# VITA-Group/FasterSeg

Measured on NVIDIA H100. Metric: fasterseg_student_fps_1024x2048, higher is better.
Workload: dtype fp16

## Files before the change

fasterseg_b200/_lib.py:

```python
import ctypes as C
import os

_HERE = os.path.dirname(os.path.abspath(__file__))
LIB_PATH = os.path.join(_HERE, "libfsb200.so")

FSB_CONV_RELU = 1
FSB_CONV_AFFINE = 2
FSB_CONV_FORCE_DIRECT = 4
FSB_CONV_STATS = 8
FSB_CONV_OUT_F32 = 16
FSB_ACT_IN_F32 = 32
FSB_CONV_X_DOWN2 = 64
FSB_CONV_Y_UP2 = 128
ABI_VERSION = 2


class FsbError(RuntimeError):
    pass


class ConvDesc(C.Structure):
    _fields_ = [(n, C.c_int32) for n in ("N", "H", "W", "Cin", "Cout", "ksize", "stride", "pad", "dil", "off_h", "off_w",
                                         "Ho", "Wo", "x_cstride", "y_cstride")] + [("flags", C.c_uint32), ("stats_C", C.c_int32),
                                                                                    ("stats_off", C.c_int32)]


class BnSel(C.Structure):
    _fields_ = [("gamma", C.c_void_p), ("beta", C.c_void_p), ("running_mean", C.c_void_p), ("running_var", C.c_void_p),
                ("num_batches_tracked", C.c_void_p), ("dgamma", C.c_void_p), ("dbeta", C.c_void_p), ("C", C.c_int32),
                ("reserved", C.c_int32)]


_P = C.c_void_p
_SIGS = {
    "fsb_abi_version": (C.c_int, []),
    "fsb_last_error_string": (C.c_char_p, []),
    "fsb_device_info": (C.c_int, [C.POINTER(C.c_int)] * 3),
    "fsb_set_pdl": (C.c_int, [C.c_int]),
    "fsb_set_option": (C.c_int, [C.c_char_p, C.c_int]),
    "fsb_get_option": (C.c_int, [C.c_char_p]),
    "fsb_conv_kernel_id": (C.c_int, [C.POINTER(ConvDesc), _P, C.c_int]),
    "fsb_conv_stats_rows": (C.c_int, [C.POINTER(ConvDesc)]),
    "fsb_stat_rows": (C.c_int, [C.c_int64]),
    "fsb_wsum_rows": (C.c_int, [C.c_int64, C.c_int]),
    "fsb_rowsum": (C.c_int, [C.c_int, _P, C.c_int, C.c_int, _P, _P]),
    "fsb_debug_set_buffer": (C.c_int, [_P]),
    "fsb_conv_packed_bytes": (C.c_size_t, [C.POINTER(ConvDesc)]),
    "fsb_pack_conv_weight": (C.c_int, [C.POINTER(ConvDesc), _P, C.c_int64, C.c_int64, _P, _P]),
    "fsb_bn_fold": (C.c_int, [C.c_int, _P, _P, _P, _P, C.c_float, _P, _P, _P, _P]),
    "fsb_conv_fwd": (C.c_int, [C.POINTER(ConvDesc), _P, _P, _P, _P, _P, _P, _P]),
    "fsb_stem_conv_nchw": (C.c_int, [C.c_int] * 4 + [_P, C.c_int, _P, _P, _P, _P, C.c_int, C.c_uint32, _P]),
    "fsb_stem_conv_u8hwc": (C.c_int, [C.c_int] * 4 + [_P, _P, _P, _P, _P, _P, C.c_int, C.c_uint32, _P]),
    "fsb_confusion_matrix": (C.c_int, [C.c_int64, _P, _P, C.c_int, C.c_int, _P, _P]),
    "fsb_bilinear_fwd": (C.c_int, [C.c_int] * 6 + [_P, C.c_int, _P, C.c_int, C.c_uint32, _P]),
    "fsb_upsample_logits_nchw": (C.c_int, [C.c_int] * 6 + [_P, C.c_int, _P, C.c_int, _P]),
    "fsb_upsample_argmax": (C.c_int, [C.c_int] * 6 + [_P, C.c_int, _P, _P]),
    "fsb_nearest_fwd": (C.c_int, [C.c_int] * 6 + [_P, C.c_int, _P, C.c_int, _P]),
    "fsb_upsample_logits_nearest_nchw": (C.c_int, [C.c_int] * 6 + [_P, C.c_int, _P, C.c_int, _P]),
    "fsb_upsample_argmax_nearest": (C.c_int, [C.c_int] * 6 + [_P, C.c_int, _P, _P]),
    "fsb_nchw_to_nhwc_f16": (C.c_int, [C.c_int] * 4 + [_P, C.c_int, _P, C.c_int, _P]),
    "fsb_nhwc_f16_to_nchw": (C.c_int, [C.c_int] * 4 + [_P, C.c_int, _P, C.c_int, _P]),
    "fsb_copy_channels": (C.c_int, [C.c_int64, C.c_int, _P, C.c_int, _P, C.c_int, _P]),
    "fsb_bn_stats": (C.c_int, [C.c_int64, C.c_int, _P, C.c_int, _P, _P]),
    "fsb_bn_finalize": (C.c_int, [C.c_int, _P, C.c_int, C.c_int, C.c_double, _P, _P, C.c_float, C.c_float, _P, _P, _P, _P, _P, _P, _P]),
    "fsb_affine_act": (C.c_int, [C.c_int64, C.c_int, _P, C.c_int, _P, _P, _P, C.c_int, C.c_uint32, _P]),
    "fsb_bn_bwd_reduce": (C.c_int, [C.c_int64, C.c_int, _P, C.c_int, _P, C.c_int, _P, C.c_int, C.c_int, _P, _P, C.c_int, _P, _P]),
    "fsb_bn_bwd_apply": (C.c_int, [C.c_int64, C.c_int, _P, C.c_int, _P, C.c_int, _P, C.c_int, C.c_int, _P, _P, _P, _P, C.c_double,
                                   C.c_int, _P, C.c_int, _P, _P, C.c_float, C.c_int, _P]),
    "fsb_bn_finalize_sel": (C.c_int, [C.c_int, _P, C.c_int, C.c_int, C.c_double, C.c_float, C.c_float, _P, _P, _P, _P, _P, _P, C.c_int, _P]),
    "fsb_affine_act_sel": (C.c_int, [C.c_int64, C.c_int, _P, C.c_int, _P, _P, _P, C.c_int, C.c_uint32, _P, _P, C.c_int, _P]),
    "fsb_bn_bwd_reduce_sel": (C.c_int, [C.c_int64, C.c_int, _P, C.c_int, _P, C.c_int, _P, C.c_int, C.c_int, _P, _P, C.c_int, _P,
                                        _P, _P, C.c_int, _P]),
    "fsb_bn_bwd_apply_sel": (C.c_int, [C.c_int64, C.c_int, _P, C.c_int, _P, C.c_int, _P, C.c_int, C.c_int, _P, _P, _P, _P, C.c_double,
                                       C.c_int, _P, C.c_int, C.c_float, _P, _P, C.c_int, _P]),
    "fsb_relu_bwd": (C.c_int, [C.c_int64, C.c_int, _P, C.c_int, _P, C.c_int, _P, C.c_int, _P]),
# ... 78 lines not shown
```

fasterseg_b200/csrc/api.cu:

```cuda
#include <stdlib.h>
#include <string.h>

#include <mutex>

#include "fsb_internal.h"

namespace fsb {

static thread_local char g_err[512] = "";
thread_local cudaError_t g_launch_err = cudaSuccess;

int set_error(int code, const char* msg) {
  snprintf(g_err, sizeof(g_err), "%s", msg);
  return code;
}
int set_cuda_error(cudaError_t e, const char* where) {
  snprintf(g_err, sizeof(g_err), "%s: %s (%s)", where, cudaGetErrorString(e), cudaGetErrorName(e));
  return FSB_ERR_CUDA;
}

static int g_pdl = -1;
bool pdl_enabled() {
  if (g_pdl < 0) {
    const char* e = getenv("FSB_PDL");
// ... 154 lines not shown
  return FSB_OK;
}

static int find_opt(const char* name) {
  if (!name) return -1;
  for (int i = 0; i < OPT_COUNT; ++i)
    if (strcmp(name, kOptNames[i]) == 0) return i;
  return -1;
}
int fsb_set_option(const char* name, int value) {
  const int i = find_opt(name);
  if (i < 0) return set_error(FSB_ERR_INVALID, "fsb_set_option: unknown option");
  opt(static_cast<Opt>(i));
  g_opts[i] = value;
  return FSB_OK;
}
int fsb_get_option(const char* name) {
  const int i = find_opt(name);
  return i < 0 ? -1 : opt(static_cast<Opt>(i));
}

int fsb_conv_stats_rows(const fsb_conv_desc* d) {
  if (check_desc(d)) return 0;
  if ((d->flags & FSB_CONV_FORCE_DIRECT) || !conv_tc_supported(d)) return stat_rows(static_cast<int64_t>(d->N) * d->Ho * d->Wo);
  return conv_tc_m_tiles(d);
}
int fsb_conv_kernel_id(const fsb_conv_desc* d, const void* y, int with_stats) {
  if (check_desc(d)) return -1;
  if ((d->flags & FSB_CONV_FORCE_DIRECT) || !conv_tc_supported(d)) return 0;
  (void)y;
  (void)with_stats;
  return conv_tc_strip(d) ? 2 : 1;
}
int fsb_stat_rows(int64_t pixels) { return stat_rows(pixels); }
int fsb_wsum_rows(int64_t pixels, int C) { return wsum_rows(pixels, C); }
int fsb_rowsum(int L, const float* src, int rows, int stride, float* out, void* stream) {
  if (L <= 0 || rows <= 0 || !src || !out || stride < L) return set_error(FSB_ERR_INVALID, "rowsum: bad argument");
  return rowsum_launch(L, src, rows, stride, out, static_cast<cudaStream_t>(stream));
}

int fsb_debug_set_buffer(void* dev_u64x128) {
  g_dbg_buffer = static_cast<unsigned long long*>(dev_u64x128);
  return FSB_OK;
}

int fsb_loss_logp_fwd(int N, int C, int Hi, int Wi, int Ho, int Wo, const void* logits, int cstride, const int64_t* target,
                      int ignore_label, float* logp_t, float* lse, void* stream) {
  return loss_logp_fwd_launch(N, C, Hi, Wi, Ho, Wo, logits, cstride, reinterpret_cast<const long long*>(target), ignore_label, logp_t, lse,
                              static_cast<cudaStream_t>(stream));
}
size_t fsb_kth_workspace_bytes(void) { return kth_workspace_bytes(); }
int fsb_kth_smallest_f32(const float* x, int64_t n, int64_t k, float* out, void* workspace, void* stream) {
  return kth_smallest_launch(x, n, k, out, workspace, static_cast<cudaStream_t>(stream));
}
int fsb_loss_rows(void) { return loss_rows(); }
int fsb_ohem_reduce(const float* logp_t, const int64_t* target, int64_t n, int ignore_label, int C, const float* thr, float* partial,
                    float* out2, void* stream) {
  return ohem_reduce_launch(logp_t, reinterpret_cast<const long long*>(target), n, ignore_label, C, thr, partial, out2,
                            static_cast<cudaStream_t>(stream));
}
int fsb_loss_ce_bwd(int N, int C, int Hi, int Wi, int Ho, int Wo, const void* logits, int cstride, const int64_t* target,
                    int ignore_label, const float* lse, const float* logp_t, const float* thr, const float* coef, void* dlogits,
                    int dcs, float gscale, int accumulate, void* stream) {
  return loss_ce_bwd_launch(N, C, Hi, Wi, Ho, Wo, logits, cstride, reinterpret_cast<const long long*>(target), ignore_label, lse, logp_t, thr,
                            coef, dlogits, dcs, gscale, accumulate, static_cast<cudaStream_t>(stream));
}
// ... 245 lines not shown
```

fasterseg_b200/csrc/conv_tc.cu:

```cuda
#include "fsb_common.cuh"
#include "fsb_internal.h"

namespace fsb {

constexpr int kTileM = 128;
constexpr int kMaxStages = 8;
constexpr int kThreads = 256;
constexpr int kAccLd = kTileM + 4;

struct ConvTcParams {
  CUtensorMap tmap_a[4];
  CUtensorMap tmap_b;
  CUtensorMap tmap_y[2];
  int tma_store;
  int tail_w;
  int taps;
  int tap_map[9];
  int tap_dh[9];
  int tap_dw[9];
  int tap_widx[9];
  int k_chunks;
  int Ho, Wo;
  int tiles_w, tiles_h;
  int tw, th;
  int win_pitch, win_rows;
  int win_sbo;
  int win_half;
  int win_stride;
  int m_half, m_grp;
  int Cout;
  int stages;
  int y_cstride;
  uint32_t flags;
  const float* scale;
  const float* shift;
  __half* y;
  float* stats;
  int stats_C;
  int stats_off;
};
// ... 8 lines not shown
__host__ __device__ constexpr uint32_t conv_tc_out_bytes() { return static_cast<uint32_t>((NT + 63) / 64) * kTileM * 128; }
template <int NT>
__host__ __device__ constexpr uint32_t conv_tc_epilogue_bytes() { return conv_tc_out_bytes<NT>() + static_cast<uint32_t>(NT) * kAccLd * 4; }


template <int BK, int NT, bool WIN, bool UP2>
__device__ __forceinline__ void conv_tc_body(const ConvTcParams& p, const CUtensorMap* tmap_up, int y_reps) {
  extern __shared__ uint8_t smem_raw[];
  __shared__ __align__(8) uint64_t full_bar[kMaxStages];
  __shared__ __align__(8) uint64_t empty_bar[kMaxStages];
  __shared__ __align__(8) uint64_t win_full[2];
  __shared__ __align__(8) uint64_t win_empty[2];
  __shared__ float s_scale[NT];
  __shared__ float s_shift[NT];

  pdl_launch_dependents();
  const int warp = threadIdx.x >> 5;
  const int lane = threadIdx.x & 31;
  constexpr uint32_t kABytes = kTileM * BK * 2;
  constexpr uint32_t kStageBytes = WIN ? NT * BK * 2 : kABytes + NT * BK * 2;
  static_assert(!WIN || BK == 64, "windows are 128B-swizzled 64-channel rows");
  uint8_t* smem = reinterpret_cast<uint8_t*>((reinterpret_cast<uintptr_t>(smem_raw) + 1023) & ~uintptr_t(1023));

  int t = blockIdx.x;
  const int tile_w = t % p.tiles_w;
  t /= p.tiles_w;
  const int tile_h = t % p.tiles_h;
  const int img = t / p.tiles_h;
  const int w0 = tile_w * p.tw;
  const int h0 = tile_h * p.th;
  const int n0 = blockIdx.y * NT;
  const int k_iters = p.taps * p.k_chunks;

  if (warp == 0 && lane == 0) {
    tma_prefetch_desc(&p.tmap_a[0]);
    tma_prefetch_desc(&p.tmap_b);
    for (int s = 0; s < p.stages; ++s) {
      mbar_init(&full_bar[s], 1);
      mbar_init(&empty_bar[s], 4);
    }
    for (int w = 0; w < 2; ++w) {
      mbar_init(&win_full[w], 1);
      mbar_init(&win_empty[w], 4);
    }
    mbar_fence_init();
  }
  pdl_wait();
  for (int c = threadIdx.x; c < NT; c += kThreads) {
    const int ch = n0 + c;
    const bool ok = ch < p.Cout;
    s_scale[c] = (ok && (p.flags & FSB_CONV_AFFINE) && p.scale) ? p.scale[ch] : 1.0f;
    s_shift[c] = (ok && (p.flags & FSB_CONV_AFFINE) && p.shift) ? p.shift[ch] : 0.0f;
  }
  __syncthreads();

  if (WIN && warp == 0) {
    uint8_t* bring = smem + 2 * p.win_stride;
    const uint32_t win_bytes = static_cast<uint32_t>(p.win_rows * p.win_pitch) * 128u;
    RingPos rp, rw;
    for (int kc = 0; kc < p.k_chunks; ++kc) {
      mbar_wait_inline(&win_empty[rw.s], rw.phase ^ 1u);
      if (elect_one()) {
        mbar_arrive_expect_tx(&win_full[rw.s], win_bytes);
        tma_load_4d(smem + rw.s * p.win_stride, &p.tmap_a[0], &win_full[rw.s], kc * BK, w0 + p.tap_dw[0], h0 + p.tap_dh[0], img);
      }
      __syncwarp();
      rw.advance(2);
      for (int tap = 0; tap < 9; ++tap) {
        mbar_wait_inline(&empty_bar[rp.s], rp.phase ^ 1u);
        if (elect_one()) {
          mbar_arrive_expect_tx(&full_bar[rp.s], kStageBytes);
          tma_load_3d(bring + rp.s * kStageBytes, &p.tmap_b, &full_bar[rp.s], kc * BK, n0, tap);
        }
        __syncwarp();
        rp.advance(p.stages);
      }
    }
  } else if (warp == 0) {
    RingPos rp;
    uint8_t* sa = smem;
    for (int tap = 0; tap < p.taps; ++tap) {
      const CUtensorMap* ma = &p.tmap_a[p.tap_map[tap]];
      const int cw = w0 + p.tap_dw[tap];
      const int chh = h0 + p.tap_dh[tap];
      const int wi = p.tap_widx[tap];
      for (int kc = 0; kc < p.k_chunks; ++kc) {
        mbar_wait_inline(&empty_bar[rp.s], rp.phase ^ 1u);
        if (elect_one()) {
          mbar_arrive_expect_tx(&full_bar[rp.s], kStageBytes);
          tma_load_4d(sa, ma, &full_bar[rp.s], kc * BK, cw, chh, img);
          tma_load_3d(sa + kABytes, &p.tmap_b, &full_bar[rp.s], kc * BK, n0, wi);
        }
        __syncwarp();
        sa += kStageBytes;
        rp.advance(p.stages);
        if (rp.s == 0) sa = smem;
      }
    }
  } else if (warp >= 4) {
    const int tw = threadIdx.x - 128;
    float acc[2][NT / 2];
#pragma unroll
    for (int h = 0; h < 2; ++h)
#pragma unroll
      for (int i = 0; i < NT / 2; ++i) acc[h][i] = 0.f;
    const uint32_t sa0 = smem_u32(smem);
    const uint64_t da0 = wgmma_desc_kmajor(sa0, BK * 2);
    const uint64_t db0 = wgmma_desc_kmajor(sa0 + kABytes, BK * 2);
    constexpr uint32_t kHalf = (64 * BK * 2) >> 4;
    if constexpr (WIN) {
      const uint64_t dw0 = wgmma_desc(sa0, 16, p.win_sbo, 128);
      const uint64_t dbr = wgmma_desc_kmajor(sa0 + 2 * p.win_stride, 128);
      const uint64_t whalf = static_cast<uint64_t>(p.win_half * 8);
      RingPos rp, rw;
      int prev = -1, prev_w = -1;
      for (int kc = 0; kc < p.k_chunks; ++kc) {
        mbar_wait_inline(&win_full[rw.s], rw.phase);
        const uint64_t dwin = dw0 + static_cast<uint64_t>(rw.s * (p.win_stride >> 4));
        for (int tap = 0; tap < 9; ++tap) {
          const int r = tap / 3, sx = tap - 3 * r;
          mbar_wait_inline(&full_bar[rp.s], rp.phase);
          wgmma_fence();
          const uint64_t da = dwin + static_cast<uint64_t>((r * p.win_pitch + sx) * 8);
          const uint64_t db = dbr + static_cast<uint64_t>(rp.s * (kStageBytes >> 4));
#pragma unroll
          for (int k = 0; k < BK / 16; ++k) {
            wgmma_f16<NT, 0>(acc[0], da + static_cast<uint64_t>(2 * k), db + static_cast<uint64_t>(2 * k));
            wgmma_f16<NT, 0>(acc[1], da + whalf + static_cast<uint64_t>(2 * k), db + static_cast<uint64_t>(2 * k));
          }
          wgmma_commit();
          wgmma_wait<1>();
          if (prev >= 0 && lane == 0) mbar_arrive(&empty_bar[prev]);
          if (tap == 0 && prev_w >= 0 && lane == 0) mbar_arrive(&win_empty[prev_w]);
// ... 15 lines not shown
        const uint64_t da = da0 + doff + static_cast<uint64_t>(2 * k), db = db0 + doff + static_cast<uint64_t>(2 * k);
        wgmma_f16<NT, 0>(acc[0], da, db);
        wgmma_f16<NT, 0>(acc[1], da + kHalf, db);
      }
      wgmma_commit();
      wgmma_wait<1>();
      if (prev >= 0 && lane == 0) mbar_arrive(&empty_bar[prev]);
      prev = rp.s;
      doff += kStageBytes >> 4;
      rp.advance(p.stages);
      if (rp.s == 0) doff = 0;
    }
    }
    wgmma_wait<0>();
    float* s_acc = reinterpret_cast<float*>(smem + conv_tc_out_bytes<NT>());
    named_bar_sync(1, 128);
    if constexpr (WIN) {
      const int row0 = wgmma_row(tw, 0);
      const int m0 = (row0 >> 3) * p.m_grp + (row0 & 7);
#pragma unroll
      for (int h = 0; h < 2; ++h) {
        float* s_h = s_acc + h * p.m_half + m0;
#pragma unroll
        for (int i = 0; i < NT / 2; ++i) s_h[wgmma_col(tw, i) * kAccLd + ((i >> 1) & 1) * p.m_grp] = acc[h][i];
      }
    } else {
#pragma unroll
      for (int h = 0; h < 2; ++h)
#pragma unroll
        for (int i = 0; i < NT / 2; ++i) s_acc[wgmma_col(tw, i) * kAccLd + 64 * h + wgmma_row(tw, i)] = acc[h][i];
    }
    named_bar_sync(1, 128);

    const int q = warp & 3;
    const int m = q * 32 + lane;
    const int oh = h0 + m / p.tw;
    const int ow = w0 + m % p.tw;
    const bool pix_ok = (oh < p.Ho) && (ow < p.Wo);
    __half* yrow = p.y + (static_cast<size_t>(img) * p.Ho * p.Wo + static_cast<size_t>(oh) * p.Wo + ow) * p.y_cstride + n0;
    const bool out_f32 = (p.flags & FSB_CONV_OUT_F32) != 0;
    float* yrow32 = reinterpret_cast<float*>(p.y) +
                    (static_cast<size_t>(img) * p.Ho * p.Wo + static_cast<size_t>(oh) * p.Wo + ow) * p.y_cstride + n0;
    const bool vec_ok = out_f32 ? ((reinterpret_cast<uintptr_t>(yrow32) & 15) == 0) : ((reinterpret_cast<uintptr_t>(yrow) & 15) == 0);
    const bool relu = (p.flags & FSB_CONV_RELU) != 0;
    const bool do_stats = (p.flags & FSB_CONV_STATS) != 0 && p.stats != nullptr;
    float* s_stat = reinterpret_cast<float*>(smem);
    for (int c0 = 0; c0 < NT; c0 += 64) {
      const int nb = min(4, (NT - c0) >> 4);
#pragma unroll
      for (int b = 0; b < 4; ++b) {
      if (b >= nb) break;
      const int c = c0 + 16 * b;
      float f[16];
#pragma unroll
      for (int j = 0; j < 16; ++j) f[j] = s_acc[(c + j) * kAccLd + m];
      if (do_stats) {
#pragma unroll
        for (int j = 0; j < 16; ++j) {
          float a = pix_ok ? f[j] : 0.f;
          float b = a * a;
#pragma unroll
          for (int o = 16; o > 0; o >>= 1) {
            a += __shfl_xor_sync(0xffffffffu, a, o);
            b += __shfl_xor_sync(0xffffffffu, b, o);
          }
          if (lane == 0) {
            s_stat[(q * 2 + 0) * NT + c + j] = a;
// ... 34 lines not shown
        if (NT - c0 >= 64) {
          *reinterpret_cast<uint4*>(slab + m * 128 + ((ch16 ^ (m & 7)) << 4)) = o0;
          *reinterpret_cast<uint4*>(slab + m * 128 + (((ch16 + 1) ^ (m & 7)) << 4)) = o1;
        } else {
          uint8_t* row = slab + m * (p.tail_w * 2) + (ch16 << 4);
          *reinterpret_cast<uint4*>(row) = o0;
          *reinterpret_cast<uint4*>(row + 16) = o1;
        }
      } else if (pix_ok) {
        const int remaining = p.Cout - (n0 + c);
        if (remaining >= 16 && vec_ok) {
          uint4 o0, o1;
          o0.x = pack_half2(f[0], f[1]);
          o0.y = pack_half2(f[2], f[3]);
          o0.z = pack_half2(f[4], f[5]);
          o0.w = pack_half2(f[6], f[7]);
          o1.x = pack_half2(f[8], f[9]);
          o1.y = pack_half2(f[10], f[11]);
          o1.z = pack_half2(f[12], f[13]);
          o1.w = pack_half2(f[14], f[15]);
          uint4* dst = reinterpret_cast<uint4*>(yrow + c);
          dst[0] = o0;
          dst[1] = o1;
        } else {
#pragma unroll
          for (int j = 0; j < 16; ++j)
            if (j < remaining) yrow[c + j] = __float2half_rn(f[j]);
        }
      }
      }
      if (p.tma_store) {
        fence_proxy_async_smem();
        named_bar_sync(1, 128);
        if (warp == 4 && lane == 0) {
          const bool full = (NT - c0) >= 64;
          tma_store_4d(&p.tmap_y[full ? 0 : 1], smem + static_cast<size_t>(c0 >> 6) * (kTileM * 128), n0 + c0, w0, h0, img);
          if constexpr (UP2)
            for (int l = 1; l < y_reps; ++l)
              tma_store_4d(&tmap_up[2 * l - 2 + (full ? 0 : 1)], smem + static_cast<size_t>(c0 >> 6) * (kTileM * 128), n0 + c0, w0,
                           h0, img);
          tma_store_commit();
        }
      }
    }
    if (p.tma_store && warp == 4 && lane == 0) tma_store_wait_read();
    if (do_stats) {
      named_bar_sync(2, 128);
      float* row = p.stats + static_cast<size_t>(blockIdx.x) * 2 * p.stats_C + p.stats_off;
      for (int ch = static_cast<int>(threadIdx.x) - 128; ch < NT; ch += 128) {
        if (n0 + ch >= p.Cout) continue;
        float a = s_stat[0 * NT + ch], b = s_stat[1 * NT + ch];
#pragma unroll
        for (int w = 1; w < 4; ++w) {
          a += s_stat[(w * 2 + 0) * NT + ch];
          b += s_stat[(w * 2 + 1) * NT + ch];
        }
        row[n0 + ch] = a;
        row[p.stats_C + n0 + ch] = b;
      }
    }
  }
  __syncthreads();
}

template <int BK, int NT, bool WIN>
__global__ void __launch_bounds__(kThreads, NT <= 64 ? 2 : 1)
conv_tc_kernel(const __grid_constant__ ConvTcParams p) {
  conv_tc_body<BK, NT, WIN, false>(p, nullptr, 1);
}

template <int BK, int NT, bool WIN>
__global__ void __launch_bounds__(kThreads, NT <= 64 ? 2 : 1)
conv_tc_up2_kernel(const __grid_constant__ ConvTcUp2Params q) {
  conv_tc_body<BK, NT, WIN, true>(q.p, q.tmap_up, q.y_reps);
}

static int encode_tiled(CUtensorMap* map, const void* base, int rank, const uint64_t* dims, const uint64_t* strides_bytes,
                        const uint32_t* box, int swizzle_bytes) {
  PFN_encodeTiled enc = get_encode_tiled();
  if (!enc) return set_error(FSB_ERR_CUDA, "cuTensorMapEncodeTiled entry point unavailable");
  cuuint32_t estr[5] = {1, 1, 1, 1, 1};
  cuuint64_t gdim[5];
  cuuint64_t gstr[5];
  cuuint32_t bdim[5];
  for (int i = 0; i < rank; ++i) {
    gdim[i] = dims[i];
    bdim[i] = box[i];
  }
  for (int i = 0; i + 1 < rank; ++i) gstr[i] = strides_bytes[i];
  CUtensorMapSwizzle sw = swizzle_bytes == 128 ? CU_TENSOR_MAP_SWIZZLE_128B
                          : (swizzle_bytes == 64 ? CU_TENSOR_MAP_SWIZZLE_64B
                                                 : (swizzle_bytes == 32 ? CU_TENSOR_MAP_SWIZZLE_32B : CU_TENSOR_MAP_SWIZZLE_NONE));
  CUresult r = enc(map, CU_TENSOR_MAP_DATA_TYPE_FLOAT16, static_cast<cuuint32_t>(rank), const_cast<void*>(base), gdim, gstr,
                   bdim, estr, CU_TENSOR_MAP_INTERLEAVE_NONE, sw, CU_TENSOR_MAP_L2_PROMOTION_L2_256B,
                   CU_TENSOR_MAP_FLOAT_OOB_FILL_NONE);
  if (r != CUDA_SUCCESS) {
    char buf[256];
    snprintf(buf, sizeof(buf),
             "cuTensorMapEncodeTiled failed (%d): rank %d dims [%llu,%llu,%llu,%llu] box [%u,%u,%u,%u] base %p stride0 %llu",
             static_cast<int>(r), rank, (unsigned long long)dims[0], (unsigned long long)dims[1],
             (unsigned long long)(rank > 2 ? dims[2] : 0), (unsigned long long)(rank > 3 ? dims[3] : 0), box[0], box[1],
             rank > 2 ? box[2] : 0, rank > 3 ? box[3] : 0, base, (unsigned long long)strides_bytes[0]);
    return set_error(FSB_ERR_CUDA, buf);
  }
  return FSB_OK;
// ... 8 lines not shown

ConvGeom conv_geom(const fsb_conv_desc* d) {
  ConvGeom g;
  g.taps = d->ksize * d->ksize;
  g.bk = (d->Cin % 64 == 0) ? 64 : 32;
  g.kpad = (d->Cin + g.bk - 1) / g.bk * g.bk;
  g.npad = (d->Cout + 15) / 16 * 16;
  return g;
}

enum ConvTcMode { kPerTap, kWindow, kStrip };
static ConvTcMode conv_tc_mode(const fsb_conv_desc* d) {
  if (d->ksize != 3 || d->stride != 1 || d->dil != 1) return kPerTap;
  const int o = opt(OPT_CONV_TC2);
  if (o == 0) return kPerTap;
  if (o == 2 && d->Cin % 64 == 0 && !(d->flags & FSB_CONV_STATS)) return kStrip;
  return kWindow;
}
bool conv_tc_strip(const fsb_conv_desc* d) { return conv_tc_mode(d) == kStrip; }

int conv_tc_m_tiles(const fsb_conv_desc* d) {
  if (conv_tc_strip(d)) return ((d->Wo + kTileM - 1) / kTileM) * d->Ho * d->N;
  const int tw = d->Wo >= 16 ? 16 : 8, th = kTileM / tw;
  return ((d->Wo + tw - 1) / tw) * ((d->Ho + th - 1) / th) * d->N;
}

int conv_tc_supported(const fsb_conv_desc* d) {
  if (d->Cin < 16 || (d->x_cstride % 8) != 0) return 0;
  if (!(d->ksize == 1 || d->ksize == 3) || !(d->stride == 1 || d->stride == 2)) return 0;
  return 1;
}

template <int BK, int NT, bool WIN = false>
static int conv_tc_run(dim3 grid, size_t smem_bytes, cudaStream_t stream, const ConvTcUp2Params& q) {
  const bool up2 = q.y_reps > 1;
  const void* kernel = up2 ? reinterpret_cast<const void*>(conv_tc_up2_kernel<BK, NT, WIN>)
                           : reinterpret_cast<const void*>(conv_tc_kernel<BK, NT, WIN>);
  if (int rc = ensure_dyn_smem(kernel, 220 * 1024, "cudaFuncSetAttribute(conv_tc)")) return rc;
  const cudaError_t e = up2 ? launch_kernel(conv_tc_up2_kernel<BK, NT, WIN>, grid, dim3(kThreads), smem_bytes, stream, q)
                            : launch_kernel(conv_tc_kernel<BK, NT, WIN>, grid, dim3(kThreads), smem_bytes, stream, q.p);
  return e == cudaSuccess ? FSB_OK : set_cuda_error(e, "conv_tc launch");
}

template <int BK, bool WIN>
static int conv_tc_run_nt(int n_tile, dim3 grid, size_t smem_bytes, cudaStream_t stream, const ConvTcUp2Params& q) {
  switch (n_tile) {
    case 16: return conv_tc_run<BK, 16, WIN>(grid, smem_bytes, stream, q);
    case 32: return conv_tc_run<BK, 32, WIN>(grid, smem_bytes, stream, q);
    case 48: return conv_tc_run<BK, 48, WIN>(grid, smem_bytes, stream, q);
    case 64: return conv_tc_run<BK, 64, WIN>(grid, smem_bytes, stream, q);
    case 96: return conv_tc_run<BK, 96, WIN>(grid, smem_bytes, stream, q);
    default: return conv_tc_run<BK, 128, WIN>(grid, smem_bytes, stream, q);
  }
}

int conv_tc_launch(const fsb_conv_desc* d, const void* x, const void* wpacked, const float* scale, const float* shift,
                   void* y, float* stats, cudaStream_t stream, const ConvTcCustom* cu, bool window_ok) {
  const ConvGeom g = conv_geom(d);
  if (cu && (d->stride != 1 || (d->flags & (FSB_CONV_OUT_F32 | FSB_CONV_STATS))))
    return set_error(FSB_ERR_INVALID, "conv_tc: custom tap tables need a stride-1 fp16 problem");
  if (cu && (d->flags & (FSB_CONV_X_DOWN2 | FSB_CONV_Y_UP2)))
    return set_error(FSB_ERR_UNSUPPORTED, "conv_tc: FSB_CONV_X_DOWN2 / FSB_CONV_Y_UP2 cannot be combined with a custom output lattice");
  if ((d->flags & FSB_CONV_X_DOWN2) && d->stride != 1)
    return set_error(FSB_ERR_UNSUPPORTED, "conv_tc: FSB_CONV_X_DOWN2 needs a stride-1 conv");
  if ((d->flags & FSB_CONV_Y_UP2) && (d->flags & (FSB_CONV_STATS | FSB_CONV_OUT_F32)))
    return set_error(FSB_ERR_UNSUPPORTED, "conv_tc: FSB_CONV_Y_UP2 cannot be combined with FSB_CONV_STATS or FSB_CONV_OUT_F32");
  if ((reinterpret_cast<uintptr_t>(x) & 15) || (reinterpret_cast<uintptr_t>(wpacked) & 15))
    return set_error(FSB_ERR_INVALID, "conv_tc: x / wpacked must be 16-byte aligned");
  ConvTcUp2Params q;
  memset(&q, 0, sizeof(q));
  ConvTcParams& p = q.p;
  const ConvTcMode mode = cu ? kPerTap : conv_tc_mode(d);
  const bool strip = mode == kStrip;
  p.taps = cu ? cu->ntaps : g.taps;
  p.Ho = cu ? cu->Ho : d->Ho;
  p.Wo = cu ? cu->Wo : d->Wo;
  p.tw = strip ? kTileM : (p.Wo >= 16 ? 16 : 8);
  p.th = kTileM / p.tw;
  p.tiles_w = (p.Wo + p.tw - 1) / p.tw;
  p.tiles_h = (p.Ho + p.th - 1) / p.th;
  for (int i = 0; i < 9; ++i) p.tap_widx[i] = i;
  p.Cout = d->Cout;
  static const int kNt[] = {16, 32, 48, 64, 96, 128};
  const int m_tiles = p.tiles_w * p.tiles_h * d->N;
  int n_tiles = (g.npad + 127) / 128;
  int ni = 0;
  while (kNt[ni] * n_tiles < g.npad) ++ni;
  int n_tile = kNt[ni];
  n_tiles = (g.npad + n_tile - 1) / n_tile;
  const int sms = sm_count();
// ... 8 lines not shown
  p.k_chunks = (g.kpad + bk - 1) / bk;
  if (win) {
    p.win_pitch = p.tw + 2;
    p.win_rows = p.th + 2;
    p.win_stride = (p.win_rows * p.win_pitch * 128 + 1023) / 1024 * 1024;
    p.m_half = 64;
    p.m_grp = 8;
    if (strip) {
      p.win_sbo = 8 * 128;
      p.win_half = 64;
    } else if (p.tw == 16) {
      p.win_sbo = p.win_pitch * 128;
      p.win_half = 8;
      p.m_half = 8;
      p.m_grp = 16;
    } else {
      p.win_sbo = p.win_pitch * 128;
      p.win_half = 8 * p.win_pitch;
    }
  }
  p.y_cstride = d->y_cstride;
  p.flags = d->flags;
  p.scale = scale;
  p.shift = shift;
  p.y = static_cast<__half*>(y);
  p.stats = stats;
  p.stats_C = d->stats_C > 0 ? d->stats_C : d->Cout;
  p.stats_off = d->stats_off;
  if ((d->flags & FSB_CONV_STATS) && stats && (d->stats_off < 0 || d->stats_off + d->Cout > p.stats_C))
    return set_error(FSB_ERR_INVALID, "conv_tc: stats_off + Cout exceeds stats_C");

  const size_t stage_bytes = (win ? 0 : static_cast<size_t>(kTileM) * bk * 2) + static_cast<size_t>(n_tile) * bk * 2;
  const int k_iters = p.taps * p.k_chunks;
  const size_t smem_budget = (n_tile == 128 || m_tiles * n_tiles <= sms || strip) ? 200 * 1024 : 100 * 1024;
  const size_t win_bytes = win ? 2 * static_cast<size_t>(p.win_stride) : 0;
  int stages = static_cast<int>((smem_budget - win_bytes) / stage_bytes);
  if (stages < 2) stages = 2;
  if (stages > kMaxStages) stages = kMaxStages;
  if (stages > k_iters) stages = k_iters;
  p.stages = stages;
  const size_t epi_bytes = n_tile == 16 ? conv_tc_epilogue_bytes<16>() : n_tile == 32 ? conv_tc_epilogue_bytes<32>()
                           : n_tile == 48 ? conv_tc_epilogue_bytes<48>() : n_tile == 64 ? conv_tc_epilogue_bytes<64>()
                           : n_tile == 96 ? conv_tc_epilogue_bytes<96>() : conv_tc_epilogue_bytes<128>();
  size_t smem_bytes = (win_bytes + stage_bytes * stages > epi_bytes ? win_bytes + stage_bytes * stages : epi_bytes) + 1024;
  const bool up2 = (d->flags & FSB_CONV_Y_UP2) != 0;
  p.tma_store = 0;
  q.y_reps = 1;
  if (!(d->flags & (FSB_CONV_OUT_F32 | FSB_CONV_STATS)) && d->Cout % 8 == 0 && d->y_cstride % 8 == 0 && (reinterpret_cast<uintptr_t>(y) & 15) == 0 &&
      n_tile % 8 == 0 && (cu || up2 || opt(OPT_NO_TMA_STORE) <= 0)) {
    const uint64_t ycs = static_cast<uint64_t>(d->y_cstride) * 2;
    uint64_t dims[4] = {static_cast<uint64_t>(d->Cout), static_cast<uint64_t>(d->Wo), static_cast<uint64_t>(d->Ho),
                        static_cast<uint64_t>(d->N)};
    uint64_t str[3] = {ycs, ycs * d->Wo, ycs * d->Wo * d->Ho};
    const uint8_t* ybase[4] = {static_cast<const uint8_t*>(y), nullptr, nullptr, nullptr};
    if (cu) {
      ybase[0] = static_cast<const uint8_t*>(cu->y_base);
      for (int i = 0; i < 4; ++i) dims[i] = cu->y_dims[i];
      for (int i = 0; i < 3; ++i) str[i] = cu->y_strides[i];
    }
    if (up2) {
      q.y_reps = 4;
      const uint64_t row = ycs * 2 * d->Wo;
      str[0] = 2 * ycs;
      str[1] = 2 * row;
      str[2] = row * 2 * d->Ho;
      for (int l = 0; l < 4; ++l) ybase[l] = static_cast<const uint8_t*>(y) + (l >> 1) * row + (l & 1) * ycs;
    }
    const uint32_t box64[4] = {64u, static_cast<uint32_t>(p.tw), static_cast<uint32_t>(p.th), 1u};
    p.tail_w = n_tile % 64;
    const uint32_t boxt[4] = {static_cast<uint32_t>(p.tail_w), static_cast<uint32_t>(p.tw), static_cast<uint32_t>(p.th), 1u};
    for (int l = 0; l < q.y_reps; ++l) {
      CUtensorMap* maps = l == 0 ? p.tmap_y : q.tmap_up + 2 * (l - 1);
      int rc = 0;
      if (n_tile >= 64) rc = encode_tiled(&maps[0], ybase[l], 4, dims, str, box64, 128);
      if (!rc && p.tail_w) rc = encode_tiled(&maps[1], ybase[l], 4, dims, str, boxt, 0);
      if (rc) return rc;
      if (n_tile < 64) maps[0] = maps[1];
// ... 34 lines not shown
    bool used[4] = {false, false, false, false};
    for (int r = 0; r < d->ksize; ++r)
      for (int s = 0; s < d->ksize; ++s) {
        const int tp = r * d->ksize + s;
        const int qh = r * d->dil - d->pad + d->off_h;
        const int qw = s * d->dil - d->pad + d->off_w;
        const int ph = ((qh % 2) + 2) % 2, pw = ((qw % 2) + 2) % 2;
        p.tap_map[tp] = ph * 2 + pw;
        p.tap_dh[tp] = floordiv(qh, 2);
        p.tap_dw[tp] = floordiv(qw, 2);
        used[ph * 2 + pw] = true;
      }
    for (int ph = 0; ph < 2; ++ph)
      for (int pw = 0; pw < 2; ++pw) {
        if (!used[ph * 2 + pw]) continue;
        const int Hp = (d->H - ph + 1) / 2, Wp = (d->W - pw + 1) / 2;
        if (Hp <= 0 || Wp <= 0) return set_error(FSB_ERR_INVALID, "conv_tc: empty parity plane");
        const uint64_t dims[4] = {static_cast<uint64_t>(d->Cin), static_cast<uint64_t>(Wp), static_cast<uint64_t>(Hp),
                                  static_cast<uint64_t>(d->N)};
        const uint64_t str[3] = {2 * cs, 2 * cs * d->W, cs * d->W * d->H};
        const __half* base = xb + (static_cast<size_t>(ph) * d->W + pw) * d->x_cstride;
        int rc = encode_tiled(&p.tmap_a[ph * 2 + pw], base, 4, dims, str, boxA, g.bk * 2);
        if (rc) return rc;
      }
    if (!used[0]) p.tmap_a[0] = p.tmap_a[p.tap_map[0]];
  }
  {
    const uint64_t dims[3] = {static_cast<uint64_t>(g.kpad), static_cast<uint64_t>(g.npad), static_cast<uint64_t>(g.taps)};
    const uint64_t str[2] = {static_cast<uint64_t>(g.kpad) * 2, static_cast<uint64_t>(g.kpad) * g.npad * 2};
    const uint32_t boxB[3] = {static_cast<uint32_t>(bk), static_cast<uint32_t>(n_tile), 1u};
    int rc = encode_tiled(&p.tmap_b, wpacked, 3, dims, str, boxB, bk * 2);
    if (rc) return rc;
  }
  const dim3 grid(static_cast<unsigned>(m_tiles), static_cast<unsigned>(n_tiles));
  if (win) return conv_tc_run_nt<64, true>(n_tile, grid, smem_bytes, stream, q);
  if (g.bk == 64) return conv_tc_run_nt<64, false>(n_tile, grid, smem_bytes, stream, q);
  return conv_tc_run_nt<32, false>(n_tile, grid, smem_bytes, stream, q);
}

}
```

fasterseg_b200/csrc/fsb_internal.h:

```cpp
#pragma once
#include <cuda.h>
#include <cuda_runtime.h>
#include <stdint.h>
#include <stdio.h>
#include <stdlib.h>
#include <string.h>

#include "../../include/fsb200.h"

namespace fsb {

int set_error(int code, const char* msg);
int set_cuda_error(cudaError_t e, const char* where);

typedef CUresult (*PFN_encodeTiled)(CUtensorMap*, CUtensorMapDataType, cuuint32_t, void*, const cuuint64_t*,
                                    const cuuint64_t*, const cuuint32_t*, const cuuint32_t*, CUtensorMapInterleave,
                                    CUtensorMapSwizzle, CUtensorMapL2promotion, CUtensorMapFloatOOBfill);
PFN_encodeTiled get_encode_tiled();

struct ConvGeom {
  int taps;
  int bk;
  int kpad;
  int npad;
// ... 34 lines not shown
  cfg.gridDim = grid;
  cfg.blockDim = block;
  cfg.dynamicSmemBytes = smem;
  cfg.stream = stream;
  cudaLaunchAttribute attr[1];
  attr[0].id = cudaLaunchAttributeProgrammaticStreamSerialization;
  attr[0].val.programmaticStreamSerializationAllowed = 1;
  cfg.attrs = attr;
  cfg.numAttrs = pdl_enabled() ? 1 : 0;
  return cudaLaunchKernelEx(&cfg, kernel, static_cast<KArgs>(args)...);
}

extern thread_local cudaError_t g_launch_err;
#define FSB_LAUNCH(kernel, grid, block, smem, stream, ...) \
  (::fsb::g_launch_err = ::fsb::launch_kernel(kernel, grid, block, smem, stream, __VA_ARGS__))
inline cudaError_t last_launch_error() {
  cudaError_t e = g_launch_err;
  g_launch_err = cudaSuccess;
  if (e == cudaSuccess) e = cudaGetLastError();
  return e;
}

struct ConvTcCustom {
  int ntaps;
  int dh[9], dw[9], widx[9];
  int Ho, Wo;
  const void* y_base;
  uint64_t y_dims[4];
  uint64_t y_strides[3];
};
int conv_tc_supported(const fsb_conv_desc* d);
bool conv_tc_strip(const fsb_conv_desc* d);
int conv_tc_launch(const fsb_conv_desc* d, const void* x, const void* wpacked, const float* scale, const float* shift,
                   void* y, float* stats, cudaStream_t stream, const ConvTcCustom* cu = nullptr, bool window_ok = true);
int conv_wgrad_tc_supported(const fsb_conv_desc* d, int dy_cstride);
int conv_wgrad_tc_launch(const fsb_conv_desc* d, const void* x, const void* dy, int dcs, float* dw, int64_t so, int64_t si,
                         float gscale, cudaStream_t stream);
int conv_direct_launch(const fsb_conv_desc* d, const void* x, const void* wpacked, const float* scale, const float* shift,
                       void* y, float* stats, cudaStream_t stream);

}
```

include/fsb200.h:

```cpp
#ifndef FSB200_H_
#define FSB200_H_

#include <stddef.h>
#include <stdint.h>

#ifdef __cplusplus
extern "C" {
#endif

#define FSB_ABI_VERSION 2

typedef enum fsb_status {
  FSB_OK = 0,
  FSB_ERR_INVALID = -1,
  FSB_ERR_CUDA = -2,
  FSB_ERR_UNSUPPORTED = -3,
  FSB_ERR_NO_DEVICE = -4
} fsb_status;

#define FSB_CONV_RELU 1u
#define FSB_CONV_AFFINE 2u
#define FSB_CONV_FORCE_DIRECT 4u
#define FSB_CONV_OUT_F32 16u
#define FSB_ACT_IN_F32 32u
// ... 20 lines not shown

typedef struct fsb_bn_sel {
  float* gamma;
  float* beta;
  float* running_mean;
  float* running_var;
  long long* num_batches_tracked;
  float* dgamma;
  float* dbeta;
  int32_t C;
  int32_t reserved;
} fsb_bn_sel;

int fsb_abi_version(void);
const char* fsb_last_error_string(void);
int fsb_device_info(int* sm_count, int* cc_major, int* cc_minor);

int fsb_set_pdl(int enabled);
int fsb_set_option(const char* name, int value);
int fsb_get_option(const char* name);

int fsb_debug_set_buffer(void* dev_u64x128);

size_t fsb_conv_packed_bytes(const fsb_conv_desc* d);
int fsb_pack_conv_weight(const fsb_conv_desc* d, const float* w, int64_t w_stride_o, int64_t w_stride_i,
                         void* packed, void* stream);
int fsb_bn_fold(int C, const float* gamma, const float* beta, const float* mean, const float* var, float eps,
                const float* conv_bias, float* scale, float* shift, void* stream);

int fsb_conv_fwd(const fsb_conv_desc* d, const void* x, const void* wpacked, const float* scale, const float* shift,
                 void* y, float* stats, void* stream);
int fsb_conv_kernel_id(const fsb_conv_desc* d, const void* y, int with_stats);
int fsb_conv_stats_rows(const fsb_conv_desc* d);

int fsb_stem_conv_nchw(int N, int H, int W, int Cout, const void* x_nchw, int x_is_f32, const float* w,
                       const float* scale, const float* shift, void* y, int y_cstride, uint32_t flags, void* stream);

int fsb_stem_conv_u8hwc(int N, int H, int W, int Cout, const uint8_t* x_hwc, const void* lut_f16, const float* w,
                        const float* scale, const float* shift, void* y, int y_cstride, uint32_t flags, void* stream);
int fsb_confusion_matrix(int64_t n, const uint8_t* pred, const void* gt, int gt_bytes, int n_cl, long long* out, void* stream);

int fsb_bilinear_fwd(int N, int C, int Hi, int Wi, int Ho, int Wo, const void* x, int x_cstride, void* y,
                     int y_cstride, uint32_t flags, void* stream);
int fsb_upsample_logits_nchw(int N, int C, int Hi, int Wi, int Ho, int Wo, const void* x, int x_cstride, void* y,
                             int out_dtype, void* stream);
int fsb_upsample_argmax(int N, int C, int Hi, int Wi, int Ho, int Wo, const void* x, int x_cstride, uint8_t* labels,
                        void* stream);
int fsb_nearest_fwd(int N, int C, int Hi, int Wi, int Ho, int Wo, const void* x, int x_cstride, void* y, int y_cstride,
                    void* stream);
int fsb_upsample_logits_nearest_nchw(int N, int C, int Hi, int Wi, int Ho, int Wo, const void* x, int x_cstride, void* y,
                                     int out_dtype, void* stream);
int fsb_upsample_argmax_nearest(int N, int C, int Hi, int Wi, int Ho, int Wo, const void* x, int x_cstride, uint8_t* labels,
                                void* stream);
int fsb_nchw_to_nhwc_f16(int N, int C, int H, int W, const void* x, int x_is_f32, void* y, int y_cstride,
                         void* stream);
int fsb_nhwc_f16_to_nchw(int N, int C, int H, int W, const void* x, int x_cstride, void* y, int y_is_f32,
                         void* stream);
int fsb_copy_channels(int64_t pixels, int C, const void* x, int x_cstride, void* y, int y_cstride, void* stream);

int fsb_stat_rows(int64_t pixels);
int fsb_rowsum(int L, const float* src, int rows, int stride, float* out, void* stream);
int fsb_bn_stats(int64_t pixels, int C, const void* x, int x_cstride, float* buf, void* stream);
int fsb_bn_finalize(int C, const float* stats, int rows, int SC, double count, const float* gamma, const float* beta, float eps,
                    float momentum, float* running_mean, float* running_var, float* scale, float* shift,
                    float* save_mean, float* save_invstd, void* stream);
int fsb_affine_act(int64_t pixels, int C, const void* x, int x_cstride, const float* scale, const float* shift,
// ... 109 lines not shown
```

Baseline: 2138.

## Shrink conv_tc CTAs to four MMA warps plus one producer warp, raise residency

New measurement: 2229, median of 6. 1.04x the previous value.

```diff
diff --git a/fasterseg_b200/_lib.py b/fasterseg_b200/_lib.py
--- a/fasterseg_b200/_lib.py
+++ b/fasterseg_b200/_lib.py
@@ -41,6 +41,7 @@
     "fsb_get_option": (C.c_int, [C.c_char_p]),
     "fsb_conv_kernel_id": (C.c_int, [C.POINTER(ConvDesc), _P, C.c_int]),
     "fsb_conv_stats_rows": (C.c_int, [C.POINTER(ConvDesc)]),
+    "fsb_conv_residency": (C.c_int, [C.POINTER(ConvDesc)]),
     "fsb_stat_rows": (C.c_int, [C.c_int64]),
     "fsb_wsum_rows": (C.c_int, [C.c_int64, C.c_int]),
     "fsb_rowsum": (C.c_int, [C.c_int, _P, C.c_int, C.c_int, _P, _P]),
diff --git a/fasterseg_b200/csrc/api.cu b/fasterseg_b200/csrc/api.cu
--- a/fasterseg_b200/csrc/api.cu
+++ b/fasterseg_b200/csrc/api.cu
@@ -210,6 +210,15 @@
   (void)with_stats;
   return conv_tc_strip(d) ? 2 : 1;
 }
+int fsb_conv_residency(const fsb_conv_desc* d) {
+  int rc = check_desc(d);
+  if (rc) return rc;
+  if ((d->flags & FSB_CONV_FORCE_DIRECT) || !conv_tc_supported(d))
+    return set_error(FSB_ERR_UNSUPPORTED, "conv_residency: the descriptor runs on the direct kernel");
+  int ctas = 0;
+  rc = conv_tc_launch(d, nullptr, nullptr, nullptr, nullptr, nullptr, nullptr, nullptr, nullptr, true, &ctas);
+  return rc ? rc : ctas;
+}
 int fsb_stat_rows(int64_t pixels) { return stat_rows(pixels); }
 int fsb_wsum_rows(int64_t pixels, int C) { return wsum_rows(pixels, C); }
 int fsb_rowsum(int L, const float* src, int rows, int stride, float* out, void* stream) {
diff --git a/fasterseg_b200/csrc/conv_tc.cu b/fasterseg_b200/csrc/conv_tc.cu
--- a/fasterseg_b200/csrc/conv_tc.cu
+++ b/fasterseg_b200/csrc/conv_tc.cu
@@ -5,7 +5,8 @@
 
 constexpr int kTileM = 128;
 constexpr int kMaxStages = 8;
-constexpr int kThreads = 256;
+constexpr int kMmaThreads = 128;
+constexpr int kThreads = kMmaThreads + 32;
 constexpr int kAccLd = kTileM + 4;
 
 struct ConvTcParams {
@@ -80,7 +81,8 @@
   const int n0 = blockIdx.y * NT;
   const int k_iters = p.taps * p.k_chunks;
 
-  if (warp == 0 && lane == 0) {
+  constexpr int kProducer = kMmaThreads / 32;
+  if (warp == kProducer && lane == 0) {
     tma_prefetch_desc(&p.tmap_a[0]);
     tma_prefetch_desc(&p.tmap_b);
     for (int s = 0; s < p.stages; ++s) {
@@ -102,7 +104,7 @@
   }
   __syncthreads();
 
-  if (WIN && warp == 0) {
+  if (WIN && warp == kProducer) {
     uint8_t* bring = smem + 2 * p.win_stride;
     const uint32_t win_bytes = static_cast<uint32_t>(p.win_rows * p.win_pitch) * 128u;
     RingPos rp, rw;
@@ -124,7 +126,7 @@
         rp.advance(p.stages);
       }
     }
-  } else if (warp == 0) {
+  } else if (warp == kProducer) {
     RingPos rp;
     uint8_t* sa = smem;
     for (int tap = 0; tap < p.taps; ++tap) {
@@ -145,8 +147,8 @@
         if (rp.s == 0) sa = smem;
       }
     }
-  } else if (warp >= 4) {
-    const int tw = threadIdx.x - 128;
+  } else {
+    const int tw = threadIdx.x;
     float acc[2][NT / 2];
 #pragma unroll
     for (int h = 0; h < 2; ++h)
@@ -228,7 +230,7 @@
     }
     named_bar_sync(1, 128);
 
-    const int q = warp & 3;
+    const int q = warp;
     const int m = q * 32 + lane;
     const int oh = h0 + m / p.tw;
     const int ow = w0 + m % p.tw;
@@ -329,7 +331,7 @@
       if (p.tma_store) {
         fence_proxy_async_smem();
         named_bar_sync(1, 128);
-        if (warp == 4 && lane == 0) {
+        if (threadIdx.x == 0) {
           const bool full = (NT - c0) >= 64;
           tma_store_4d(&p.tmap_y[full ? 0 : 1], smem + static_cast<size_t>(c0 >> 6) * (kTileM * 128), n0 + c0, w0, h0, img);
           if constexpr (UP2)
@@ -340,11 +342,11 @@
         }
       }
     }
-    if (p.tma_store && warp == 4 && lane == 0) tma_store_wait_read();
+    if (p.tma_store && threadIdx.x == 0) tma_store_wait_read();
     if (do_stats) {
       named_bar_sync(2, 128);
       float* row = p.stats + static_cast<size_t>(blockIdx.x) * 2 * p.stats_C + p.stats_off;
-      for (int ch = static_cast<int>(threadIdx.x) - 128; ch < NT; ch += 128) {
+      for (int ch = static_cast<int>(threadIdx.x); ch < NT; ch += kMmaThreads) {
         if (n0 + ch >= p.Cout) continue;
         float a = s_stat[0 * NT + ch], b = s_stat[1 * NT + ch];
 #pragma unroll
@@ -360,14 +362,16 @@
   __syncthreads();
 }
 
+__host__ __device__ constexpr int conv_tc_residency(int nt) { return nt <= 64 ? 3 : 2; }
+
 template <int BK, int NT, bool WIN>
-__global__ void __launch_bounds__(kThreads, NT <= 64 ? 2 : 1)
+__global__ void __launch_bounds__(kThreads, conv_tc_residency(NT))
 conv_tc_kernel(const __grid_constant__ ConvTcParams p) {
   conv_tc_body<BK, NT, WIN, false>(p, nullptr, 1);
 }
 
 template <int BK, int NT, bool WIN>
-__global__ void __launch_bounds__(kThreads, NT <= 64 ? 2 : 1)
+__global__ void __launch_bounds__(kThreads, conv_tc_residency(NT))
 conv_tc_up2_kernel(const __grid_constant__ ConvTcUp2Params q) {
   conv_tc_body<BK, NT, WIN, true>(q.p, q.tmap_up, q.y_reps);
 }
@@ -442,30 +446,36 @@
 }
 
 template <int BK, int NT, bool WIN = false>
-static int conv_tc_run(dim3 grid, size_t smem_bytes, cudaStream_t stream, const ConvTcUp2Params& q) {
+static int conv_tc_run(dim3 grid, size_t smem_bytes, cudaStream_t stream, const ConvTcUp2Params& q, int* residency) {
   const bool up2 = q.y_reps > 1;
   const void* kernel = up2 ? reinterpret_cast<const void*>(conv_tc_up2_kernel<BK, NT, WIN>)
                            : reinterpret_cast<const void*>(conv_tc_kernel<BK, NT, WIN>);
   if (int rc = ensure_dyn_smem(kernel, 220 * 1024, "cudaFuncSetAttribute(conv_tc)")) return rc;
+  if (residency) {
+    const cudaError_t e = cudaOccupancyMaxActiveBlocksPerMultiprocessor(residency, kernel, kThreads, smem_bytes);
+    return e == cudaSuccess ? FSB_OK : set_cuda_error(e, "cudaOccupancyMaxActiveBlocksPerMultiprocessor(conv_tc)");
+  }
   const cudaError_t e = up2 ? launch_kernel(conv_tc_up2_kernel<BK, NT, WIN>, grid, dim3(kThreads), smem_bytes, stream, q)
                             : launch_kernel(conv_tc_kernel<BK, NT, WIN>, grid, dim3(kThreads), smem_bytes, stream, q.p);
   return e == cudaSuccess ? FSB_OK : set_cuda_error(e, "conv_tc launch");
 }
 
 template <int BK, bool WIN>
-static int conv_tc_run_nt(int n_tile, dim3 grid, size_t smem_bytes, cudaStream_t stream, const ConvTcUp2Params& q) {
+static int conv_tc_run_nt(int n_tile, dim3 grid, size_t smem_bytes, cudaStream_t stream, const ConvTcUp2Params& q, int* residency) {
   switch (n_tile) {
-    case 16: return conv_tc_run<BK, 16, WIN>(grid, smem_bytes, stream, q);
-    case 32: return conv_tc_run<BK, 32, WIN>(grid, smem_bytes, stream, q);
-    case 48: return conv_tc_run<BK, 48, WIN>(grid, smem_bytes, stream, q);
-    case 64: return conv_tc_run<BK, 64, WIN>(grid, smem_bytes, stream, q);
-    case 96: return conv_tc_run<BK, 96, WIN>(grid, smem_bytes, stream, q);
-    default: return conv_tc_run<BK, 128, WIN>(grid, smem_bytes, stream, q);
-  }
-}
+    case 16: return conv_tc_run<BK, 16, WIN>(grid, smem_bytes, stream, q, residency);
+    case 32: return conv_tc_run<BK, 32, WIN>(grid, smem_bytes, stream, q, residency);
+    case 48: return conv_tc_run<BK, 48, WIN>(grid, smem_bytes, stream, q, residency);
+    case 64: return conv_tc_run<BK, 64, WIN>(grid, smem_bytes, stream, q, residency);
+    case 96: return conv_tc_run<BK, 96, WIN>(grid, smem_bytes, stream, q, residency);
+    default: return conv_tc_run<BK, 128, WIN>(grid, smem_bytes, stream, q, residency);
+  }
+}
+
+static size_t conv_tc_static_smem(int n_tile) { return (2 * kMaxStages + 4) * 8 + static_cast<size_t>(n_tile) * 2 * 4; }
 
 int conv_tc_launch(const fsb_conv_desc* d, const void* x, const void* wpacked, const float* scale, const float* shift,
-                   void* y, float* stats, cudaStream_t stream, const ConvTcCustom* cu, bool window_ok) {
+                   void* y, float* stats, cudaStream_t stream, const ConvTcCustom* cu, bool window_ok, int* residency) {
   const ConvGeom g = conv_geom(d);
   if (cu && (d->stride != 1 || (d->flags & (FSB_CONV_OUT_F32 | FSB_CONV_STATS))))
     return set_error(FSB_ERR_INVALID, "conv_tc: custom tap tables need a stride-1 fp16 problem");
@@ -540,7 +550,9 @@
 
   const size_t stage_bytes = (win ? 0 : static_cast<size_t>(kTileM) * bk * 2) + static_cast<size_t>(n_tile) * bk * 2;
   const int k_iters = p.taps * p.k_chunks;
-  const size_t smem_budget = (n_tile == 128 || m_tiles * n_tiles <= sms || strip) ? 200 * 1024 : 100 * 1024;
+  const int grid_res = (m_tiles * n_tiles + sms - 1) / sms;
+  const int res = strip ? 1 : (grid_res < conv_tc_residency(n_tile) ? grid_res : conv_tc_residency(n_tile));
+  const size_t smem_budget = res <= 1 ? 200 * 1024 : 227 * 1024 / res - conv_tc_static_smem(n_tile) - 2 * 1024;
   const size_t win_bytes = win ? 2 * static_cast<size_t>(p.win_stride) : 0;
   int stages = static_cast<int>((smem_budget - win_bytes) / stage_bytes);
   if (stages < 2) stages = 2;
@@ -551,6 +563,17 @@
                            : n_tile == 48 ? conv_tc_epilogue_bytes<48>() : n_tile == 64 ? conv_tc_epilogue_bytes<64>()
                            : n_tile == 96 ? conv_tc_epilogue_bytes<96>() : conv_tc_epilogue_bytes<128>();
   size_t smem_bytes = (win_bytes + stage_bytes * stages > epi_bytes ? win_bytes + stage_bytes * stages : epi_bytes) + 1024;
+  if (smem_bytes < smem_budget + 1024) smem_bytes = smem_budget + 1024;
+  const dim3 grid(static_cast<unsigned>(m_tiles), static_cast<unsigned>(n_tiles));
+  auto run = [&]() {
+    if (win) return conv_tc_run_nt<64, true>(n_tile, grid, smem_bytes, stream, q, residency);
+    if (g.bk == 64) return conv_tc_run_nt<64, false>(n_tile, grid, smem_bytes, stream, q, residency);
+    return conv_tc_run_nt<32, false>(n_tile, grid, smem_bytes, stream, q, residency);
+  };
+  if (residency) {
+    q.y_reps = (d->flags & FSB_CONV_Y_UP2) ? 4 : 1;
+    return run();
+  }
   const bool up2 = (d->flags & FSB_CONV_Y_UP2) != 0;
   p.tma_store = 0;
   q.y_reps = 1;
@@ -651,10 +674,7 @@
     int rc = encode_tiled(&p.tmap_b, wpacked, 3, dims, str, boxB, bk * 2);
     if (rc) return rc;
   }
-  const dim3 grid(static_cast<unsigned>(m_tiles), static_cast<unsigned>(n_tiles));
-  if (win) return conv_tc_run_nt<64, true>(n_tile, grid, smem_bytes, stream, q);
-  if (g.bk == 64) return conv_tc_run_nt<64, false>(n_tile, grid, smem_bytes, stream, q);
-  return conv_tc_run_nt<32, false>(n_tile, grid, smem_bytes, stream, q);
-}
-
-}
+  return run();
+}
+
+}
diff --git a/fasterseg_b200/csrc/fsb_internal.h b/fasterseg_b200/csrc/fsb_internal.h
--- a/fasterseg_b200/csrc/fsb_internal.h
+++ b/fasterseg_b200/csrc/fsb_internal.h
@@ -90,7 +90,8 @@
 int conv_tc_supported(const fsb_conv_desc* d);
 bool conv_tc_strip(const fsb_conv_desc* d);
 int conv_tc_launch(const fsb_conv_desc* d, const void* x, const void* wpacked, const float* scale, const float* shift,
-                   void* y, float* stats, cudaStream_t stream, const ConvTcCustom* cu = nullptr, bool window_ok = true);
+                   void* y, float* stats, cudaStream_t stream, const ConvTcCustom* cu = nullptr, bool window_ok = true,
+                   int* residency = nullptr);
 int conv_wgrad_tc_supported(const fsb_conv_desc* d, int dy_cstride);
 int conv_wgrad_tc_launch(const fsb_conv_desc* d, const void* x, const void* dy, int dcs, float* dw, int64_t so, int64_t si,
                          float gscale, cudaStream_t stream);
diff --git a/include/fsb200.h b/include/fsb200.h
--- a/include/fsb200.h
+++ b/include/fsb200.h
@@ -76,6 +76,7 @@
                  void* y, float* stats, void* stream);
 int fsb_conv_kernel_id(const fsb_conv_desc* d, const void* y, int with_stats);
 int fsb_conv_stats_rows(const fsb_conv_desc* d);
+int fsb_conv_residency(const fsb_conv_desc* d);
 
 int fsb_stem_conv_nchw(int N, int H, int W, int Cout, const void* x_nchw, int x_is_f32, const float* w,
                        const float* scale, const float* shift, void* y, int y_cstride, uint32_t flags, void* stream);
```
